# arcosoph/nanowakeword

Hardware: AMD Instinct MI355X
Metric: clips/sec (1 s @16 kHz PCM->logits) (higher is better)
Workload: dtype f32; 1 GPU; cnn head on (101,64) log-mel, batch=4096/GPU, 1 s 16 kHz mono int16 clips, 64-mel 25 ms/10 ms center frontend, fused STFT+mel HIP kernel, fp32; clips_per_gpu=4096, n_samples=16000, parallelism=batch-split x1

## Files before the change

### nanowakeword_amd/csrc/fe_steps.h

```cpp
#pragma once
#include <math.h>
#include <stdint.h>

#if defined(__HIPCC__)
#include <hip/hip_runtime.h>
#define NWW_HD __host__ __device__ __forceinline__
typedef float2 nww_c32;
#else
#define NWW_HD inline
struct nww_c32 { float x, y; };
#endif

#define FE_NFFT 400
#define FE_M 200
#define FE_BINS 201
#define FE_PSTRIDE 209
#define FE_MAX_MELS 128
#define FE_MAX_MELW 640

NWW_HD nww_c32 c_make(float x, float y) { nww_c32 r; r.x = x; r.y = y; return r; }
NWW_HD nww_c32 c_add(nww_c32 a, nww_c32 b) { return c_make(a.x + b.x, a.y + b.y); }
NWW_HD nww_c32 c_sub(nww_c32 a, nww_c32 b) { return c_make(a.x - b.x, a.y - b.y); }
NWW_HD nww_c32 c_mul(nww_c32 a, nww_c32 b) { return c_make(a.x * b.x - a.y * b.y, a.x * b.y + a.y * b.x); }
NWW_HD nww_c32 c_mul_negi(nww_c32 a) { return c_make(a.y, -a.x); }
// ... 126 lines not shown
NWW_HD float fe_s4(int f, int j, const FeTables* tb, const float* pw) {
    const float* p = pw + f * FE_PSTRIDE + tb->mel_lo[j];
    const float* w = tb->melw + tb->mel_off[j];
    const int n = tb->mel_cnt[j];
    float acc = 0.0f;
    for (int i = 0; i < n; ++i) acc = fmaf(p[i], w[i], acc);
    return acc;
}

NWW_HD float fe_db(float mel, float amin, float mult) {
    return mult * log10f(fmaxf(mel, amin));
}

NWW_HD int fe_reflect(int s, int N) {
    if (s < 0) s = -s;
    if (s >= N) s = 2 * (N - 1) - s;
    return s;
}

#define FE2_G 8
#define FE2_FRAME_DW 400
#define FE2_PSHIFT(f) (4 * ((f) >> 1))
#define FE2_STAGE_OFF 216
#define FE2_MAX_TILES 8
#define FE2_MAX_STEPS 512

#define FE2_CHUNK 8
#define FE2_MAX_CHUNKS 64
struct Fe2MelPlan {
    int32_t ntiles;
    int32_t total_steps;
    int32_t nchunks;
    int32_t tile_k0[FE2_MAX_TILES];
    int32_t tile_nsteps[FE2_MAX_TILES];
    int32_t tile_first[FE2_MAX_TILES];
    uint32_t chunk_meta[FE2_MAX_CHUNKS];
    float b[FE2_MAX_STEPS * 64];
};

NWW_HD void fe2_s1(const uint32_t s[8], const nww_c32 win[8], const nww_c32 tw[7], nww_c32 z[8]) {
#pragma unroll
    for (int n1 = 0; n1 < 8; ++n1)
        z[n1] = c_make((float)(int16_t)(s[n1] & 0xffffu) * win[n1].x, (float)(int16_t)(s[n1] >> 16) * win[n1].y);
    dft8(z);
#pragma unroll
    for (int k1 = 1; k1 < 8; ++k1) z[k1] = c_mul(z[k1], tw[k1 - 1]);
}

NWW_HD float fe2_mel_planned(const Fe2MelPlan* pl, const float* p, int j) {
    const int t = j >> 4, n = j & 15;
    const int k0 = pl->tile_k0[t], ns = pl->tile_nsteps[t];
    const float* b = pl->b + (size_t)pl->tile_first[t] * 64 + n;
    float acc[2] = {0.0f, 0.0f};
    for (int s = 0; s < ns; ++s)
        for (int kk = 0; kk < 4; ++kk) acc[s & 1] = fmaf(p[k0 + 4 * s + kk], b[s * 64 + kk * 16], acc[s & 1]);
    return acc[0] + acc[1];
}
```

### nanowakeword_amd/csrc/fe_tables.cpp

```cpp
#include "fe_tables.h"
#include <cmath>
#include <cstring>

static const double kPi = 3.14159265358979323846;

void fe_default_window(int win_length, std::vector<float>& window) {
    window.resize(win_length);
    for (int n = 0; n < win_length; ++n)
        window[n] = (float)(0.5 - 0.5 * std::cos(2.0 * kPi * n / win_length));
}

void fe_default_melfb(const FeParams& p, std::vector<float>& fb) {
    const int n_freqs = p.n_fft / 2 + 1;
    fb.assign((size_t)n_freqs * p.n_mels, 0.f);
    const double m_min = 2595.0 * std::log10(1.0 + (double)p.f_min / 700.0);
    const double m_max = 2595.0 * std::log10(1.0 + (double)p.f_max / 700.0);
    std::vector<double> f_pts(p.n_mels + 2);
    for (int i = 0; i < p.n_mels + 2; ++i) {
        const double m = m_min + (m_max - m_min) * i / (p.n_mels + 1);
        f_pts[i] = 700.0 * (std::pow(10.0, m / 2595.0) - 1.0);
    }
    const double nyq = (double)(p.sample_rate / 2);
    for (int k = 0; k < n_freqs; ++k) {
        const double f = nyq * k / (n_freqs - 1);
// ... 66 lines not shown
            for (int n = 0; n < 16; ++n) {
                const int j = 16 * t + n;
                if (j < p.n_mels && fb[(size_t)k * p.n_mels + j] != 0.f) { if (k < lo) lo = k; if (k > hi) hi = k; }
            }
        if (hi < 0) { lo = 0; hi = 0; }
        int ns = (hi - lo + 1 + 3) / 4;
        ns = (ns + FE2_CHUNK - 1) / FE2_CHUNK * FE2_CHUNK;
        if (first + ns > FE2_MAX_STEPS || (first + ns) / FE2_CHUNK > FE2_MAX_CHUNKS) return "mel filterbank is too dense for the MFMA plan";
        for (int c = 0; c < ns / FE2_CHUNK; ++c)
            pl->chunk_meta[first / FE2_CHUNK + c] =
                (uint32_t)(lo + 4 * FE2_CHUNK * c) | ((uint32_t)t << 12) | ((c == ns / FE2_CHUNK - 1) ? 1u << 16 : 0u);
        pl->tile_k0[t] = lo; pl->tile_nsteps[t] = ns; pl->tile_first[t] = first;
        for (int s = 0; s < ns; ++s)
            for (int l = 0; l < 64; ++l) {
                const int k = lo + 4 * s + (l >> 4), j = 16 * t + (l & 15);
                pl->b[(size_t)(first + s) * 64 + l] = (k < FE_BINS && j < p.n_mels) ? fb[(size_t)k * p.n_mels + j] : 0.f;
            }
        first += ns;
    }
    pl->total_steps = first;
    pl->nchunks = first / FE2_CHUNK;
    return "";
}
```

### nanowakeword_amd/csrc/fe_tables.h

```cpp
#pragma once
#include <string>
#include <vector>
#include "fe_steps.h"

struct FeParams {
    int sample_rate = 16000, n_fft = 400, win_length = 400, hop = 160, n_mels = 64, center = 1;
    float f_min = 0.f, f_max = 8000.f, amin = 1e-10f, db_mult = 10.f;
};

void fe_default_window(int win_length, std::vector<float>& window);
void fe_default_melfb(const FeParams& p, std::vector<float>& fb);

std::string fe_build_tables(const FeParams& p, const float* window, const float* fb, FeTables* out);

std::string fe2_build_mel_plan(const FeParams& p, const float* fb, Fe2MelPlan* out);

int fe_num_frames(const FeParams& p, int n_samples);
```

### nanowakeword_amd/csrc/frontend.h

```cpp
#pragma once
#include <hip/hip_runtime.h>
#include "fe_tables.h"

int fe2_lds_bytes(int waves, int mel_mode);
struct Fe2Sub {
    int nr = 0;
    int t0[4] = {0, 0, 0, 0}, t1[4] = {0, 0, 0, 0};
    int gend[4] = {0, 0, 0, 0};
    int ring_rows = 0, row0 = 0;
    size_t out_clip_stride = 0;
};
bool fe2_subset_supported(const FeParams& p, int mel_mode);
hipError_t fe2_launch(const int16_t* d_pcm, size_t row_stride, int B, int N, int T, const FeParams& p,
                      const FeTables* d_tables, const Fe2MelPlan* d_plan, float* d_db, float* d_mel, int frames_major,
                      int mel_mode, int max_taps, int block, int max_grid, hipStream_t stream, const Fe2Sub* subset = nullptr);
```

### nanowakeword_amd/csrc/frontend2.hip

```cpp
#include <hip/hip_runtime.h>
#include <stdlib.h>
#include "fe_steps.h"
#include "frontend.h"
#include "layers.h"

typedef float f32x4 __attribute__((ext_vector_type(4)));

struct Fe2MelLds {
    uint32_t desc[FE_MAX_MELS];
    float w[FE_MAX_MELW];
};

__device__ __forceinline__ void fe2_wave_sync() {
    __builtin_amdgcn_fence(__ATOMIC_RELEASE, "wavefront");
    __builtin_amdgcn_wave_barrier();
    __builtin_amdgcn_fence(__ATOMIC_ACQUIRE, "wavefront");
}

__device__ __forceinline__ void fe2_load_column(const int16_t* __restrict__ x, int base, int n2, uint32_t v[8]) {
    const uint32_t* p = reinterpret_cast<const uint32_t*>(x + base) + n2;
#pragma unroll
    for (int n1 = 0; n1 < 8; ++n1) v[n1] = p[25 * n1];
}

__device__ __forceinline__ float fe2_db(float mel, float amin, float mult, float floor_db) {
    const float db = (mult * 0.30102999566398120f) * __log2f(fmaxf(mel, amin));
    return mel > amin ? db : floor_db;
}

#define FE2_PARAMS                                                                                                      \
    const int16_t *__restrict__ pcm, size_t row_stride, int B, int N, int T, int ngroups, int hop, int pad, int n_mels,    \
        float amin, float db_mult, float floor_db, const FeTables *__restrict__ gtb, const Fe2MelPlan *__restrict__ plan,  \
        float *__restrict__ out_db, float *__restrict__ out_mel, int frames_major, int dbg, int gsz, Fe2Sub sub
#define FE2_ARGS pcm, row_stride, B, N, T, ngroups, hop, pad, n_mels, amin, db_mult, floor_db, gtb, plan, out_db, out_mel, frames_major, dbg, gsz, sub
template <int MEL, int FAST_OUT, int MAXT, bool RING>
__device__ __forceinline__ void fe2_wave_body(FE2_PARAMS) {
    extern __shared__ __attribute__((aligned(16))) char smem[];
    constexpr int MFMA_MEL = MEL == 1;
    const int lane = threadIdx.x & 63;
    const int wv = __builtin_amdgcn_readfirstlane((int)(threadIdx.x >> 6));
    const int nwv = blockDim.x >> 6;
    const int tb_bytes = MEL == 0 ? (int)sizeof(Fe2MelLds) : 0;
    Fe2MelLds* mt = reinterpret_cast<Fe2MelLds*>(smem);
    float* slab = reinterpret_cast<float*>(smem + tb_bytes) + wv * (FE2_G * FE2_FRAME_DW);
    if (MEL == 0) {
        for (int i = threadIdx.x; i < FE_MAX_MELS; i += blockDim.x)
            mt->desc[i] = (uint32_t)gtb->mel_lo[i] | ((uint32_t)gtb->mel_cnt[i] << 8) | ((uint32_t)gtb->mel_off[i] << 16);
        for (int i = threadIdx.x; i < FE_MAX_MELW; i += blockDim.x) mt->w[i] = gtb->melw[i];
        __syncthreads();
    }
    const int n2 = lane % 25, slot = lane / 25;
    nww_c32 win[8], tw[7];
#pragma unroll
    for (int n1 = 0; n1 < 8; ++n1) win[n1] = gtb->win2[25 * n1 + n2];
#pragma unroll
    for (int k1 = 1; k1 < 8; ++k1) tw[k1 - 1] = gtb->tw200[k1 * 25 + n2];
    const int k3a = lane, k3b = 64 + lane;
    const bool has_b = k3b <= 100;
    const nww_c32 twa = gtb->tw400[k3a], twb = gtb->tw400[has_b ? k3b : 100];
    const int ia2 = k3a ? FE_M - k3a : 0;
    const int f2 = lane >> 3, k1_2 = lane & 7;
    int co_off[4];
#pragma unroll
    for (int r = 0; r < 4; ++r) {
        const int i = 4 * lane + 256 * r, f = i / n_mels, j = i - f * n_mels;
        co_off[r] = f * FE2_FRAME_DW + FE2_STAGE_OFF + FE2_PSHIFT(f) + j;
    }
    const int mel_l5 = lane & 31;
    const int mel_j = (lane & 32) + ((mel_l5 < 4) ? mel_l5 : (mel_l5 < 12) ? 12 + mel_l5 : (mel_l5 < 16) ? mel_l5 - 8 : (mel_l5 < 20) ? 8 + mel_l5
                                     : (mel_l5 < 28) ? mel_l5 - 12 : mel_l5);
    float wreg[MAXT];
    int mel_lo_lane = 0;
    if (MEL == 2) {
        const int j = min(mel_j, n_mels - 1);
        const int lo = gtb->mel_lo[j], sh4 = lo & 3;
        mel_lo_lane = lo - sh4;
        const int cnt = mel_j < n_mels ? gtb->mel_cnt[j] : 0, off = gtb->mel_off[j];
#pragma unroll
        for (int i = 0; i < MAXT; ++i) wreg[i] = (i >= sh4 && i - sh4 < cnt) ? gtb->melw[off + i - sh4] : 0.0f;
    }
    const int mel_nchunks = MFMA_MEL ? plan->nchunks : 0;
    const uint32_t mel_meta = MFMA_MEL ? plan->chunk_meta[lane] : 0u;
    const bool aligned = ((reinterpret_cast<uintptr_t>(pcm) | (row_stride * sizeof(int16_t))) & 3) == 0;

    const int total = B * ngroups;
    const int stride = gridDim.x * nwv;
    uint32_t cur[8];
    auto geom = [&](int item, int& b, int& t0, int& nf) {
        b = item / ngroups;
        const int g = item - b * ngroups;
        if (!RING || sub.nr == 0) {
            t0 = g * gsz;
            nf = min(gsz, T - t0);
        } else {
            int r = 0;
            while (r + 1 < sub.nr && g >= sub.gend[r]) ++r;
            t0 = sub.t0[r] + (g - (r ? sub.gend[r - 1] : 0)) * gsz;
            nf = min(gsz, sub.t1[r] - t0);
        }
    };
    auto interior = [&](int t0, int nf) {
        const int s0 = t0 * hop - pad;
// ... 40 lines not shown
#pragma unroll
                    for (int n1 = 0; n1 < 8; ++n1) nxt[n1] = span[((fn * hop) >> 1) + n2 + 25 * n1];
                }
            }
            if (slot < 2 && f < nf && !(dbg & 1)) {
                nww_c32 z[8];
                fe2_s1(cur, win, tw, z);
                nww_c32* y = reinterpret_cast<nww_c32*>(slab + f * FE2_FRAME_DW) + n2;
#pragma unroll
                for (int k1 = 0; k1 < 8; ++k1) y[k1 * 25] = z[k1];
            }
#pragma unroll
            for (int n1 = 0; n1 < 8; ++n1) cur[n1] = nxt[n1];
        }
        fe2_wave_sync();
        if (f2 < nf && !(dbg & 2)) {
            nww_c32* zf = reinterpret_cast<nww_c32*>(slab + f2 * FE2_FRAME_DW);
            const nww_c32* row = zf + k1_2 * 25;
            nww_c32* dst = zf + k1_2;
            dft25<true>([&](int i) { return row[i]; }, [&](int i, nww_c32 v) { dst[8 * i] = v; });
        }
        fe2_wave_sync();
        if (item + stride < total) prefetch_first(item + stride);
        if (!(dbg & 4)) {
            const nww_c32* z0 = reinterpret_cast<const nww_c32*>(slab);
            nww_c32 a1 = z0[k3a], b1 = z0[ia2], a2 = z0[has_b ? k3b : 0], b2 = z0[has_b ? FE_M - k3b : 0];
#pragma unroll
            for (int f = 0; f < FE2_G; ++f) {
                if (f >= nf) break;
                nww_c32 na1 = a1, nb1 = b1, na2 = a2, nb2 = b2;
                if (f + 1 < FE2_G) {
                    const nww_c32* zn = reinterpret_cast<const nww_c32*>(slab + (f + 1) * FE2_FRAME_DW);
                    na1 = zn[k3a]; nb1 = zn[ia2]; na2 = zn[has_b ? k3b : 0]; nb2 = zn[has_b ? FE_M - k3b : 0];
                }
                float pa1, pb1, pa2, pb2;
                fe_s3_core(a1, b1, twa, &pa1, &pb1);
                fe_s3_core(a2, b2, twb, &pa2, &pb2);
                float* p = slab + f * FE2_FRAME_DW + FE2_PSHIFT(f);
                p[k3a] = pa1;
                p[FE_M - k3a] = pb1;
                if (has_b) { p[k3b] = pa2; p[FE_M - k3b] = pb2; }
                a1 = na1; b1 = nb1; a2 = na2; b2 = nb2;
            }
        }
        fe2_wave_sync();
        if (!(dbg & 8)) {
// ... 37 lines not shown
                                            const size_t o = ((size_t)b * n_mels + j) * T + t0 + f;
                                            if (out_db) out_db[o] = db;
                                            if (out_mel) out_mel[o] = m;
                                        }
                                    }
                                }
                            }
                        }
                        acc0 = f32x4{0.f, 0.f, 0.f, 0.f};
                        acc1 = f32x4{0.f, 0.f, 0.f, 0.f};
                    }
                };
                float a0[FE2_CHUNK], b0[FE2_CHUNK], a1[FE2_CHUNK], b1[FE2_CHUNK];
                const int last = mel_nchunks - 1;
                load_chunk(0, a0, b0);
#pragma unroll 1
                for (int c = 0; c < mel_nchunks; c += 2) {
                    load_chunk(min(c + 1, last), a1, b1);
                    run_chunk(c, a0, b0);
                    load_chunk(min(c + 2, last), a0, b0);
                    if (c + 1 < mel_nchunks) run_chunk(c + 1, a1, b1);
                }
            } else if (MEL == 2) {
                const float* p0 = slab + mel_lo_lane;
#pragma unroll 1
                for (int f = 0; f < nf; f += 2) {
                    const float* pa = p0 + f * FE2_FRAME_DW + FE2_PSHIFT(f);
                    const float* pb = pa + FE2_FRAME_DW;
                    float ma = 0.0f, mb = 0.0f;
#pragma unroll
                    for (int i = 0; i < MAXT; i += 4) {
                        const float4 a4 = *reinterpret_cast<const float4*>(__builtin_assume_aligned(pa + i, 16));
                        const float4 b4 = *reinterpret_cast<const float4*>(__builtin_assume_aligned(pb + i, 16));
                        ma = fmaf(a4.x, wreg[i], ma); mb = fmaf(b4.x, wreg[i], mb);
                        ma = fmaf(a4.y, wreg[i + 1], ma); mb = fmaf(b4.y, wreg[i + 1], mb);
                        ma = fmaf(a4.z, wreg[i + 2], ma); mb = fmaf(b4.z, wreg[i + 2], mb);
                        ma = fmaf(a4.w, wreg[i + 3], ma); mb = fmaf(b4.w, wreg[i + 3], mb);
                    }
                    if (mel_j < n_mels) {
                        const float da = fe2_db(ma, amin, db_mult, floor_db), db2 = fe2_db(mb, amin, db_mult, floor_db);
                        if (FAST_OUT) {
                            float* st = slab + f * FE2_FRAME_DW + FE2_STAGE_OFF + FE2_PSHIFT(f) + mel_j;
                            st[0] = da;
                            st[FE2_FRAME_DW] = db2;
                        } else {
#pragma unroll
                            for (int q = 0; q < 2; ++q) {
                                const int fq = f + q;
                                const float m = q ? mb : ma, db = q ? db2 : da;
                                if (fq < nf) {
                                    if (frames_major) {
                                        slab[fq * FE2_FRAME_DW + FE2_STAGE_OFF + FE2_PSHIFT(fq) + mel_j] = db;
                                        if (out_mel) out_mel[((size_t)b * T + t0 + fq) * n_mels + mel_j] = m;
                                    } else {
                                        const size_t o = ((size_t)b * n_mels + mel_j) * T + t0 + fq;
                                        if (out_db) out_db[o] = db;
                                        if (out_mel) out_mel[o] = m;
                                    }
                                }
                            }
                        }
                    }
                }
            } else {
                const int f = lane & 7;
                if (f < nf) {
                    const float* prow = slab + f * FE2_FRAME_DW + FE2_PSHIFT(f);
                    for (int j = lane >> 3; j < n_mels; j += 8) {
                        const uint32_t d = mt->desc[j];
                        const float* p = prow + (d & 0xffu);
                        const float* w = mt->w + (d >> 16);
                        const int n = (d >> 8) & 0xffu;
                        float m = 0.0f;
                        for (int i = 0; i < n; ++i) m = fmaf(p[i], w[i], m);
                        const float db = fe2_db(m, amin, db_mult, floor_db);
                        if (frames_major) {
                            slab[f * FE2_FRAME_DW + FE2_STAGE_OFF + FE2_PSHIFT(f) + j] = db;
                            if (out_mel) out_mel[((size_t)b * T + t0 + f) * n_mels + j] = m;
                        } else {
                            const size_t o = ((size_t)b * n_mels + j) * T + t0 + f;
                            if (out_db) out_db[o] = db;
// ... 24 lines not shown
                }
            } else {
                for (int i = lane; i < cnt; i += 64) {
                    const int f = i / n_mels, j = i - f * n_mels;
                    dst[i] = slab[f * FE2_FRAME_DW + FE2_STAGE_OFF + FE2_PSHIFT(f) + j];
                }
            }
            }
        }
        fe2_wave_sync();
    }
}

template <int MEL, int FAST_OUT, int MAXT, bool RING = false>
__global__ void __launch_bounds__(256, 3) fe2_wave_kernel(FE2_PARAMS) { fe2_wave_body<MEL, FAST_OUT, MAXT, RING>(FE2_ARGS); }

bool fe2_subset_supported(const FeParams& p, int mel_mode) { return mel_mode != 0 && (p.n_mels & 3) == 0; }

int fe2_lds_bytes(int waves, int mel_mode) {
    return waves * FE2_G * FE2_FRAME_DW * 4 + (mel_mode == 0 ? (int)sizeof(Fe2MelLds) : 0);
}

hipError_t fe2_launch(const int16_t* d_pcm, size_t row_stride, int B, int N, int T, const FeParams& p,
                      const FeTables* d_tables, const Fe2MelPlan* d_plan, float* d_db, float* d_mel, int frames_major,
                      int mel_mode, int max_taps, int block, int max_grid, hipStream_t stream, const Fe2Sub* subset) {
    if (block < 64 || block > 1024 || (block & 63)) return hipErrorInvalidValue;
    const int nwv = block / 64;
    Fe2Sub sub = subset ? *subset : Fe2Sub{};
    if (sub.nr < 0 || sub.nr > 4) return hipErrorInvalidValue;
    if ((sub.nr || sub.ring_rows) && !(frames_major && d_db && !d_mel && (p.n_mels & 3) == 0)) return hipErrorInvalidValue;
    if (sub.ring_rows && (sub.ring_rows < T || sub.row0 < 0 || sub.row0 >= sub.ring_rows)) return hipErrorInvalidValue;
    auto count_groups = [&](int g) {
        if (sub.nr == 0) return (T + g - 1) / g;
        int n = 0;
        for (int r = 0; r < sub.nr; ++r) { n += (sub.t1[r] - sub.t0[r] + g - 1) / g; sub.gend[r] = n; }
        return n;
    };
    for (int r = 0; r < sub.nr; ++r)
        if (sub.t0[r] < 0 || sub.t1[r] <= sub.t0[r] || sub.t1[r] > T) return hipErrorInvalidValue;
    int ngroups = count_groups(FE2_G);
    int mode = mel_mode;
    if (mode == 2 && (p.n_mels > 64 || max_taps > 25)) mode = 1;
    const int lds = fe2_lds_bytes(nwv, mode);
    const int fast = (frames_major && d_db && !d_mel) ? 1 : 0;
    const bool ring = sub.nr > 0 || sub.ring_rows > 0;
    if (ring && (mode == 0 || !fast)) return hipErrorInvalidValue;
    auto kern = mode == 0 ? fe2_wave_kernel<0, 0, 1>
              : mode == 1 ? (ring ? fe2_wave_kernel<1, 1, 1, true> : fast ? fe2_wave_kernel<1, 1, 1> : fe2_wave_kernel<1, 0, 1>)
              : max_taps <= 17 ? (ring ? fe2_wave_kernel<2, 1, 20, true> : fast ? fe2_wave_kernel<2, 1, 20> : fe2_wave_kernel<2, 0, 20>)
                               : (ring ? fe2_wave_kernel<2, 1, 28, true> : fast ? fe2_wave_kernel<2, 1, 28> : fe2_wave_kernel<2, 0, 28>);
    const void* fn = reinterpret_cast<const void*>(kern);
    {
        hipError_t e = nww_allow_lds(fn, (size_t)lds);
        if (e != hipSuccess) return e;
    }
#ifdef NWW_ABLATION
    static const int dbg = [] { const char* e = getenv("NWW_FE_DBG"); return e ? atoi(e) : 0; }();
#else
    const int dbg = 0;
#endif
    const int small_g = 2;
    int gsz = FE2_G;
    if (mode == 2 && small_g >= 2 && small_g < FE2_G && (small_g % 2) == 0 && (long long)B * ngroups * 4 <= (long long)max_grid * nwv) {
        gsz = small_g;
        ngroups = count_groups(gsz);
    }
    const long long total = (long long)B * ngroups;
    long long need = (total + nwv - 1) / nwv;
    int grid = (int)(need < max_grid ? need : max_grid);
    if (grid < 1) grid = 1;
    const int pad = p.center ? FE_NFFT / 2 : 0;
    hipLaunchKernelGGL(kern, dim3(grid), dim3(block), lds, stream, d_pcm, row_stride, B, N, T, ngroups, p.hop, pad, p.n_mels,
                       p.amin, p.db_mult, p.db_mult * log10f(p.amin), d_tables, d_plan, d_db, d_mel, frames_major, dbg, gsz, sub);
    return hipGetLastError();
}
```

### nanowakeword_amd/csrc/nww_api.hip

```cpp
#include "nww_internal.h"

static hipEvent_t prof_event(nww_handle* h) {
    hipEvent_t e = nullptr;
    if (!h->event_pool.empty()) { e = h->event_pool.back(); h->event_pool.pop_back(); return e; }
    if (hipEventCreate(&e) != hipSuccess) return nullptr;
    return e;
}
void nww_prof_mark(nww_handle* h, hipStream_t s, int id_of_next) {
    if (!h->profiling || !h->prof_active) return;
    hipEvent_t e = prof_event(h);
    if (!e) return;
    (void)hipEventRecord(e, s);
    h->prof_runs.back().push_back(e);
    h->prof_ids.back().push_back(id_of_next);
}
void nww_prof_begin(nww_handle* h) {
    if (!h->profiling) return;
    h->prof_active = (h->prof_counter++ % h->prof_period) == 0;
    if (!h->prof_active) return;
    h->prof_runs.emplace_back();
    h->prof_ids.emplace_back();
}

static thread_local std::string g_create_err;
// ... 98 lines not shown
        if (p) (void)hipFree(p);
    h->d_ws = nullptr; h->d_pcm = nullptr; h->d_logmel = nullptr; h->d_feats = nullptr; h->d_emb = nullptr;
    h->d_hid = nullptr; h->d_logits = nullptr; h->d_probs = nullptr; h->d_splitk = nullptr; h->cap_B = 0; h->cap_N = 0;
}

extern "C" int nww_stream_close(nww_handle* h);

extern "C" int nww_emb_close(nww_handle* h);
extern "C" int nww_comm_destroy(nww_handle* h);
extern "C" int nww_destroy(nww_handle* h) {
    if (!h) return NWW_OK;
    (void)hipSetDevice(h->cfg.device);
    free_ws(h);
    nww_stream_close(h);
    nww_emb_close(h);
    nww_comm_destroy(h);
    if (h->pin_in) (void)hipHostFree(h->pin_in);
    if (h->pin_out) (void)hipHostFree(h->pin_out);
    if (h->d_weights) (void)hipFree(h->d_weights);
    for (auto& kv : h->x3_weights) (void)hipFree(kv.second);
    for (void* d : h->packed_weights) (void)hipFree(d);
    if (h->d_tables) (void)hipFree(h->d_tables);
    if (h->d_melplan) (void)hipFree(h->d_melplan);
    if (h->own_stream) (void)hipStreamDestroy(h->own_stream);
    for (auto& run : h->prof_runs) for (auto e : run) (void)hipEventDestroy(e);
    for (auto e : h->event_pool) (void)hipEventDestroy(e);
    delete h;
    return NWW_OK;
}

extern "C" int nww_num_tensors(const nww_handle* h) { return h ? (int)h->keys.size() : 0; }

extern "C" int nww_tensor_info(const nww_handle* h, int32_t i, const char** key, int64_t* shape4, int32_t* ndim) {
    if (!h || i < 0 || i >= (int)h->keys.size()) return NWW_ERR_INVALID;
    const std::string& k = h->keys[i];
    const HostTensor& t = h->tensors.at(k);
    if (key) *key = k.c_str();
    if (ndim) *ndim = (int)t.shape.size();
    if (shape4) for (size_t d = 0; d < 4; ++d) shape4[d] = d < t.shape.size() ? t.shape[d] : 1;
    return NWW_OK;
}

extern "C" int nww_load_tensor(nww_handle* h, const char* key, const void* host, const int64_t* shape, int32_t ndim,
                               int32_t dtype) {
    if (!h || !key || !host || !shape || ndim < 0) return fail(h, NWW_ERR_INVALID, "nww_load_tensor: null argument");
    if (h->finalized) return fail(h, NWW_ERR_STATE, "nww_load_tensor('%s') after nww_finalize", key);
// ... 147 lines not shown
    if (d_probs && r.need_sigmoid) {
        nww_prof_mark(h, s, id);
        hipError_t e = launch_unary(r.logits, d_probs, (size_t)B, ACT_SIGMOID, s);
        if (e != hipSuccess) return fail(h, NWW_ERR_HIP, "launch 'sigmoid' failed: %s", hipGetErrorString(e));
    }
    nww_prof_mark(h, s, -1);
    if (done_armed) *done_armed = r.done_armed;
    return NWW_OK;
}

int nww_check_run(nww_handle* h, int B) {
    if (!h) return NWW_ERR_INVALID;
    if (!h->finalized) return fail(h, NWW_ERR_STATE, "model not finalized: call nww_finalize after loading the state_dict");
    if (B <= 0) return fail(h, NWW_ERR_INVALID, "batch must be positive (got %d)", B);
    return NWW_OK;
}

int nww_frontend_on_dev(nww_handle* h, const int16_t* d_pcm, int B, int N, float* d_db, float* d_mel, int frames_major,
                        hipStream_t s, int* frames_out, size_t row_stride, const Fe2Sub* sub) {
    const int T = fe_num_frames(h->fe, N);
    if (T <= 0) return fail(h, NWW_ERR_INVALID, "clip of %d samples is too short for n_fft=%d (center=%d)", N, h->fe.n_fft, h->fe.center);
    if (frames_out) *frames_out = T;
    static const int mel_env = 2;
    hipError_t e = fe2_launch(d_pcm, row_stride ? row_stride : (size_t)N, B, N, T, h->fe, h->d_tables, h->d_melplan, d_db, d_mel, frames_major, mel_env, h->mel_max_taps, 256, h->cu_count * 3, s, sub);
    if (e != hipSuccess) return fail(h, NWW_ERR_HIP, "frontend launch failed: %s", hipGetErrorString(e));
    return NWW_OK;
}

extern "C" int nww_frontend_dev(nww_handle* h, const int16_t* d_pcm, int32_t B, int32_t N, float* d_logmel,
                                int32_t frames_major, void* stream) {
    int rc = nww_check_run(h, B);
    if (rc) return rc;
    if (!d_pcm || !d_logmel) return fail(h, NWW_ERR_INVALID, "null device pointer");
    HIP_TRY(h, hipSetDevice(h->cfg.device));
    return nww_frontend_on_dev(h, d_pcm, B, N, d_logmel, nullptr, frames_major, stream ? (hipStream_t)stream : h->own_stream, nullptr);
}

int nww_forward_pcm_on_dev(nww_handle* h, const int16_t* d_pcm, int B, int N, float* d_logits, float* d_probs, hipStream_t s,
                           size_t row_stride, unsigned int* done_flag, unsigned int done_seq, bool* done_armed) {
    const nww_config& c = h->cfg;
    const int T = fe_num_frames(h->fe, N);
    if (T <= 0) return fail(h, NWW_ERR_INVALID, "clip of %d samples is too short for n_fft=%d (center=%d)", N, h->fe.n_fft, h->fe.center);
    const int rows = c.mel_major_features ? c.n_mels : T, cols = c.mel_major_features ? T : c.n_mels;
    if (rows != c.in_rows || cols != c.in_cols)
        return fail(h, NWW_ERR_SHAPE, "frontend yields (%d,%d) features for %d samples but the head was built for input_shape=(%d,%d)",
                    rows, cols, N, c.in_rows, c.in_cols);
    int rc = nww_ensure_ws(h, B, N);
// ... 205 lines not shown
```

### nanowakeword_amd/csrc/nww_internal.h

```cpp
#pragma once
#include <hip/hip_runtime.h>
#include <atomic>
#include <cmath>
#include <cstdarg>
#include <cstdio>
#include <cstdlib>
#include <cstring>
#include <functional>
#include <map>
#include <string>
#include <vector>

#include "../../include/nww.h"
#include "fe_tables.h"
#include "frontend.h"
#include "layers.h"
#include "trunk.h"
#include "ffn_x3.h"
#include "lin_x3.h"
#include "attn_x3.h"
#include "dual_x3.h"
#include "emb_stream.h"
#include "tcn_x3.h"

// ... 29 lines not shown
    bool need_sigmoid = true;
    unsigned int* done_flag = nullptr; unsigned int done_seq = 0; bool done_armed = false;
    float* splitk_ws = nullptr; size_t splitk_floats = 0; int cu_count = 256;
    struct { bool active = false; int out_id = 0, parts = 0; size_t stride = 0; const float *bias = nullptr, *alpha = nullptr, *beta = nullptr; int act = 0; } deferred;
};


struct X3Key {
    const float* w; int fmt; float scale;
    bool operator<(const X3Key& o) const { return w != o.w ? w < o.w : fmt != o.fmt ? fmt < o.fmt : scale < o.scale; }
};

struct nww_handle {
    bool e2e_transposed = false;
    nww_config cfg;
    FeParams fe;
    std::string err;
    std::vector<std::string> keys;
    std::map<std::string, HostTensor> tensors;
    bool finalized = false;
    float* d_weights = nullptr;
    FeTables* d_tables = nullptr;
    Fe2MelPlan* d_melplan = nullptr;
    int mel_max_taps = 0;
    hipStream_t own_stream = nullptr;
    std::vector<Step> plan;
    size_t buf_per_clip[6] = {0, 0, 0, 0, 0, 0};
    int cap_B = 0, cap_N = 0;
    bool trunk_blocked = false;
    int cap_rows = 0;
    float* d_ws = nullptr;
    int16_t* d_pcm = nullptr;
    float* d_logmel = nullptr;
    float* d_feats = nullptr;
    float* d_emb = nullptr;
    float* d_hid = nullptr;
    float* d_logits = nullptr;
    float* d_probs = nullptr;
    float* d_splitk = nullptr;
    int16_t* d_ring = nullptr; int16_t* d_chunk = nullptr;
    std::string plan_error;
    bool clamps_features = false;
    bool x_stride_ok = false;
    bool stream_conv = false;
    int stream_H = 0, stream_W = 0;
    bool inc_fe = false, inc_conv = false, primed = false;
    float* d_lm_ring = nullptr; int lm_rows = 0, lm_pos = 0, lm_shift = 0, fe_edge_l = 0, fe_edge_r = 0;
// ... 66 lines not shown
```

### nanowakeword_amd/csrc/nww_plan.hip

```cpp
#include "nww_internal.h"
#include "bc_chain.h"

const Knobs& nww_knobs() {
    static const Knobs k = [] {
        auto env = [](const char* name, int d) { const char* e = getenv(name); return e ? atoi(e) : d; };
        Knobs r;
        r.trunk = env("NWW_TRUNK", 1); r.conv_mfma = env("NWW_CONV_MFMA", 1); r.conv3_x3 = env("NWW_CONV3_X3", 1);
        r.gemm_x3 = env("NWW_GEMM_X3", 1); r.lin_x3 = env("NWW_LIN_X3", 1); r.ffn_fused = env("NWW_FFN_FUSED", 1);
        r.attn_fused = env("NWW_ATTN_FUSED", 1); r.mha_mfma = env("NWW_MHA_MFMA", 1); r.bc_front = env("NWW_BC_FRONT", 1);
        r.bc_chain = env("NWW_BC_CHAIN", 1); r.tail = env("NWW_TAIL", 1); r.stream_inc = env("NWW_STREAM_INC", 3);
        r.f16_range_log2 = env("NWW_F16_RANGE_LOG2", 16);
        return r;
    }();
    return k;
}

namespace {
using Shape = std::vector<int64_t>;
struct SpecBuilder {
    std::vector<std::string>& keys;
    std::map<std::string, HostTensor>& t;
    void add(const std::string& k, Shape s) { keys.push_back(k); t[k].shape = std::move(s); }
    void lin(const std::string& p, int out, int in) { add(p + ".weight", {out, in}); add(p + ".bias", {out}); }
    void ln(const std::string& p, int d) { add(p + ".weight", {d}); add(p + ".bias", {d}); }
// ... 643 lines not shown
    }
    HIP_TRY(h, hipMalloc(&h->d_weights, (total + 4) * sizeof(float)));
    for (auto& kv : h->tensors) {
        if (!kv.second.loaded || kv.first.rfind("frontend.", 0) == 0) continue;
        HIP_TRY(h, hipMemcpy(h->d_weights + kv.second.dev_off, kv.second.data.data(), kv.second.data.size() * sizeof(float),
                             hipMemcpyHostToDevice));
    }
    return NWW_OK;
}

int build_frontend_tables(nww_handle* h) {
    std::vector<float> win, fb;
    auto wi = h->tensors.find("frontend.window");
    if (wi != h->tensors.end() && wi->second.loaded) win = wi->second.data; else fe_default_window(h->fe.win_length, win);
    auto fi = h->tensors.find("frontend.mel_fb");
    if (fi != h->tensors.end() && fi->second.loaded) fb = fi->second.data; else fe_default_melfb(h->fe, fb);
    FeTables tb;
    const std::string e = fe_build_tables(h->fe, win.data(), fb.data(), &tb);
    if (!e.empty()) return fail(h, NWW_ERR_INVALID, "frontend tables: %s", e.c_str());
    const size_t tbytes = (sizeof(FeTables) + 15) & ~(size_t)15;
    HIP_TRY(h, hipMalloc(&h->d_tables, tbytes));
    HIP_TRY(h, hipMemset(h->d_tables, 0, tbytes));
    HIP_TRY(h, hipMemcpy(h->d_tables, &tb, sizeof(FeTables), hipMemcpyHostToDevice));
    h->mel_max_taps = 0;
    for (int j = 0; j < h->fe.n_mels; ++j) h->mel_max_taps = tb.mel_cnt[j] > h->mel_max_taps ? tb.mel_cnt[j] : h->mel_max_taps;
    std::vector<Fe2MelPlan> plan(1);
    const std::string e2 = fe2_build_mel_plan(h->fe, fb.data(), plan.data());
    if (!e2.empty()) return fail(h, NWW_ERR_INVALID, "frontend mel plan: %s", e2.c_str());
    HIP_TRY(h, hipMalloc(&h->d_melplan, sizeof(Fe2MelPlan)));
    HIP_TRY(h, hipMemcpy(h->d_melplan, plan.data(), sizeof(Fe2MelPlan), hipMemcpyHostToDevice));
    return NWW_OK;
}

bool add_attn_x3(PlanCtx& p, const std::string& q, int hb, int T, int D, int NH) {
    if (!(nww_knobs().attn_fused && p.h->f16 && p.h->conv_products == 6 && attn_x3_supported(T, D, NH))) return false;
    const float *iw = p.W(q + ".attention.in_proj_weight"), *ib = p.W(q + ".attention.in_proj_bias");
    const float *ow = p.W(q + ".attention.out_proj.weight"), *ob = p.W(q + ".attention.out_proj.bias");
    const auto hiw = f16_fetch(p.h, iw, (size_t)3 * D * D), how = f16_fetch(p.h, ow, (size_t)D * D);
    const float ws_in = f16_wscale(hiw), ws_out = f16_wscale(how);
    auto l1max = [&](int r0) {
        double worst = 0;
        for (int r = r0; r < r0 + D; ++r) {
            double t = 0;
            for (int k = 0; k < D; ++k) t += std::fabs((double)hiw[(size_t)r * D + k]);
            worst = std::fmax(worst, t);
        }
        return worst;
    };
// ... 771 lines not shown
```

Before: 9.300 million clips/s.

## Pack two mel filters per lane with host-built pair plan for register mel stage

```diff
diff --git a/nanowakeword_amd/csrc/fe_steps.h b/nanowakeword_amd/csrc/fe_steps.h
--- a/nanowakeword_amd/csrc/fe_steps.h
+++ b/nanowakeword_amd/csrc/fe_steps.h
@@ -172,6 +172,7 @@
 #define FE2_FRAME_DW 400
 #define FE2_PSHIFT(f) (4 * ((f) >> 1))
 #define FE2_STAGE_OFF 216
+#define FE2_STAGE_SPARE 100
 #define FE2_MAX_TILES 8
 #define FE2_MAX_STEPS 512
 
@@ -188,6 +189,19 @@
     float b[FE2_MAX_STEPS * 64];
 };
 
+#define FE2_PAIR_WAVES 12
+#define FE2_PAIR_MAXW 32
+struct Fe2PairPlan {
+    int32_t sx, sy;
+    int32_t maxt;
+    int32_t lane_a[64], lane_b[64];
+    int32_t lane_par[64];
+    int32_t lane_flex[64];
+    int32_t bin_f[64], bin_x[64], bin_y[64];
+    float w[64][FE2_PAIR_MAXW];
+    int32_t rt[FE2_PAIR_WAVES][64][8];
+};
+
 NWW_HD void fe2_s1(const uint32_t s[8], const nww_c32 win[8], const nww_c32 tw[7], nww_c32 z[8]) {
 #pragma unroll
     for (int n1 = 0; n1 < 8; ++n1)
diff --git a/nanowakeword_amd/csrc/fe_tables.cpp b/nanowakeword_amd/csrc/fe_tables.cpp
--- a/nanowakeword_amd/csrc/fe_tables.cpp
+++ b/nanowakeword_amd/csrc/fe_tables.cpp
@@ -112,3 +112,115 @@
     pl->nchunks = first / FE2_CHUNK;
     return "";
 }
+
+int fe2_filter_chunks(const FeTables* tb, int j) {
+    const int cnt = tb->mel_cnt[j];
+    return cnt > 0 ? ((tb->mel_lo[j] & 3) + cnt + 3) / 4 : 0;
+}
+
+namespace {
+struct Pair { int a, b; };
+
+bool pair_filters(const FeTables* tb, int n_mels, int sx, int sy, std::vector<Pair>& pairs) {
+    std::vector<int> order(n_mels), ch(n_mels);
+    for (int j = 0; j < n_mels; ++j) { order[j] = j; ch[j] = fe2_filter_chunks(tb, j); }
+    for (int i = 1; i < n_mels; ++i)
+        for (int k = i; k > 0 && ch[order[k]] > ch[order[k - 1]]; --k) { const int t = order[k]; order[k] = order[k - 1]; order[k - 1] = t; }
+    std::vector<char> used(n_mels, 0);
+    pairs.clear();
+    for (int i = 0; i < n_mels; ++i) {
+        const int a = order[i];
+        if (used[a]) continue;
+        used[a] = 1;
+        if (ch[a] > sx + 1) return false;
+        const int room = ch[a] == sx + 1 ? sy : sy + 1;
+        int b = -1;
+        for (int k = i + 1; k < n_mels && b < 0; ++k)
+            if (!used[order[k]] && ch[order[k]] <= room) b = order[k];
+        if (b >= 0) used[b] = 1;
+        pairs.push_back({a, b});
+    }
+    return pairs.size() <= 32;
+}
+
+int lane_position(int lane) {
+    const int l5 = lane & 31;
+    return (lane & 32) + (l5 < 4 ? l5 : l5 < 12 ? 12 + l5 : l5 < 16 ? l5 - 8 : l5 < 20 ? 8 + l5 : l5 < 28 ? l5 - 12 : l5);
+}
+}
+
+std::string fe2_build_pair_plan(const FeParams& p, const FeTables* tb, Fe2PairPlan* pl) {
+    std::memset(pl, 0, sizeof(*pl));
+    if (p.n_mels <= 0 || p.n_mels > 64) return "the register-filter mel stage takes n_mels <= 64";
+    const int n = p.n_mels;
+    static const int shapes[2][2] = {{4, 1}, {6, 1}};
+    std::vector<Pair> pairs;
+    int sx = 0, sy = 0, maxt = 0;
+    for (int s = 0; s < 2 && !maxt; ++s)
+        if (pair_filters(tb, n, shapes[s][0], shapes[s][1], pairs)) { sx = shapes[s][0]; sy = shapes[s][1]; maxt = 4 * (1 + sx + sy); }
+    if (!maxt) {
+        int widest = 0;
+        for (int j = 0; j < n; ++j) widest = fe2_filter_chunks(tb, j) > widest ? fe2_filter_chunks(tb, j) : widest;
+        bool ok = false;
+        for (int steps = 1; steps <= 2 * widest + 1 && !ok; ++steps)
+            for (sy = 0; sy < steps && !ok; ++sy) { sx = steps - 1 - sy; ok = sx >= sy && pair_filters(tb, n, sx, sy, pairs); if (ok) break; }
+        if (!ok) return "no lane assignment for the mel filterbank";
+    }
+    pl->sx = sx; pl->sy = sy; pl->maxt = maxt;
+    for (size_t i = 1; i < pairs.size(); ++i)
+        for (size_t k = i; k > 0 && tb->mel_lo[pairs[k].a] < tb->mel_lo[pairs[k - 1].a]; --k) { const Pair t = pairs[k]; pairs[k] = pairs[k - 1]; pairs[k - 1] = t; }
+    auto weight = [&](int j, int bin) {
+        const int i = bin - tb->mel_lo[j];
+        return (j >= 0 && i >= 0 && i < tb->mel_cnt[j]) ? tb->melw[tb->mel_off[j] + i] : 0.0f;
+    };
+    for (int lane = 0; lane < 64; ++lane) {
+        const int pos = lane_position(lane), g = pos >> 4, pi = (g >> 1) * 16 + (pos & 15);
+        pl->lane_a[lane] = pl->lane_b[lane] = -1;
+        pl->lane_par[lane] = g & 1;
+        const int fa = (g & 1) * FE2_FRAME_DW, fb = FE2_FRAME_DW - fa;
+        auto addresses = [&]() {
+            const int a = pl->lane_a[lane], b = pl->lane_b[lane], flex = pl->lane_flex[lane];
+            for (int v = 0; v < FE2_PAIR_WAVES; ++v) {
+                const int slab = v * FE2_G * FE2_FRAME_DW;
+                int32_t* r = pl->rt[v][lane];
+                r[0] = 4 * (slab + pl->bin_f[lane] + (flex ? fa : fb));
+                r[1] = 4 * (slab + pl->bin_x[lane] + fa);
+                r[2] = 4 * (slab + pl->bin_y[lane] + fb);
+                r[3] = (g & 1) | (flex ? (int32_t)0x80000000u : 0);
+                r[4] = 4 * (slab + fa + FE2_STAGE_OFF + (a >= 0 ? a : FE2_STAGE_SPARE));
+                r[5] = 4 * (slab + fb + FE2_STAGE_OFF + (b >= 0 ? b : FE2_STAGE_SPARE));
+                r[6] = a; r[7] = b;
+            }
+        };
+        if (pi >= (int)pairs.size()) { addresses(); continue; }
+        const int a = pairs[pi].a, b = pairs[pi].b;
+        const int flex = fe2_filter_chunks(tb, a) == sx + 1;
+        const int a0 = tb->mel_lo[a] & ~3, b0 = b >= 0 ? tb->mel_lo[b] & ~3 : 0;
+        pl->lane_a[lane] = a; pl->lane_b[lane] = b; pl->lane_flex[lane] = flex;
+        pl->bin_f[lane] = flex ? a0 : b0;
+        pl->bin_x[lane] = flex ? a0 + 4 : a0;
+        pl->bin_y[lane] = flex ? b0 : b0 + 4;
+        addresses();
+        if (!maxt) continue;
+        float* w = pl->w[lane];
+        for (int i = 0; i < 4; ++i) w[i] = flex ? weight(a, a0 + i) : (b >= 0 ? weight(b, b0 + i) : 0.0f);
+        for (int i = 0; i < 4 * sx; ++i) w[4 + i] = weight(a, pl->bin_x[lane] + i);
+        for (int i = 0; i < 4 * sy; ++i) w[4 + 4 * sx + i] = b >= 0 ? weight(b, pl->bin_y[lane] + i) : 0.0f;
+    }
+    return "";
+}
+
+extern "C" int fe2_pair_plan_query(int n_mels, const float* fb, int32_t* out) {
+    FeParams p; p.n_mels = n_mels;
+    std::vector<float> w, f;
+    fe_default_window(p.win_length, w);
+    if (!fb) { fe_default_melfb(p, f); fb = f.data(); }
+    FeTables tb;
+    std::vector<Fe2PairPlan> pl(1);
+    if (!fe_build_tables(p, w.data(), fb, &tb).empty() || !fe2_build_pair_plan(p, &tb, pl.data()).empty()) return -1;
+    out[0] = pl[0].sx; out[1] = pl[0].sy; out[2] = pl[0].maxt;
+    for (int l = 0; l < 64; ++l) {
+        out[3 + l] = pl[0].lane_a[l]; out[67 + l] = pl[0].lane_b[l]; out[131 + l] = pl[0].lane_par[l]; out[195 + l] = pl[0].lane_flex[l];
+    }
+    return 0;
+}
diff --git a/nanowakeword_amd/csrc/fe_tables.h b/nanowakeword_amd/csrc/fe_tables.h
--- a/nanowakeword_amd/csrc/fe_tables.h
+++ b/nanowakeword_amd/csrc/fe_tables.h
@@ -15,4 +15,7 @@
 
 std::string fe2_build_mel_plan(const FeParams& p, const float* fb, Fe2MelPlan* out);
 
+std::string fe2_build_pair_plan(const FeParams& p, const FeTables* tb, Fe2PairPlan* out);
+int fe2_filter_chunks(const FeTables* tb, int j);
+
 int fe_num_frames(const FeParams& p, int n_samples);
diff --git a/nanowakeword_amd/csrc/frontend.h b/nanowakeword_amd/csrc/frontend.h
--- a/nanowakeword_amd/csrc/frontend.h
+++ b/nanowakeword_amd/csrc/frontend.h
@@ -12,5 +12,5 @@
 };
 bool fe2_subset_supported(const FeParams& p, int mel_mode);
 hipError_t fe2_launch(const int16_t* d_pcm, size_t row_stride, int B, int N, int T, const FeParams& p,
-                      const FeTables* d_tables, const Fe2MelPlan* d_plan, float* d_db, float* d_mel, int frames_major,
-                      int mel_mode, int max_taps, int block, int max_grid, hipStream_t stream, const Fe2Sub* subset = nullptr);
+                      const FeTables* d_tables, const Fe2MelPlan* d_plan, const Fe2PairPlan* d_pair, int pair_maxt, float* d_db, float* d_mel,
+                      int frames_major, int mel_mode, int block, int max_grid, hipStream_t stream, const Fe2Sub* subset = nullptr);
diff --git a/nanowakeword_amd/csrc/frontend2.hip b/nanowakeword_amd/csrc/frontend2.hip
--- a/nanowakeword_amd/csrc/frontend2.hip
+++ b/nanowakeword_amd/csrc/frontend2.hip
@@ -31,8 +31,8 @@
 #define FE2_PARAMS                                                                                                      \
     const int16_t *__restrict__ pcm, size_t row_stride, int B, int N, int T, int ngroups, int hop, int pad, int n_mels,    \
         float amin, float db_mult, float floor_db, const FeTables *__restrict__ gtb, const Fe2MelPlan *__restrict__ plan,  \
-        float *__restrict__ out_db, float *__restrict__ out_mel, int frames_major, int dbg, int gsz, Fe2Sub sub
-#define FE2_ARGS pcm, row_stride, B, N, T, ngroups, hop, pad, n_mels, amin, db_mult, floor_db, gtb, plan, out_db, out_mel, frames_major, dbg, gsz, sub
+        const Fe2PairPlan *__restrict__ pair, float *__restrict__ out_db, float *__restrict__ out_mel, int frames_major, int dbg, int gsz, Fe2Sub sub
+#define FE2_ARGS pcm, row_stride, B, N, T, ngroups, hop, pad, n_mels, amin, db_mult, floor_db, gtb, plan, pair, out_db, out_mel, frames_major, dbg, gsz, sub
 template <int MEL, int FAST_OUT, int MAXT, bool RING>
 __device__ __forceinline__ void fe2_wave_body(FE2_PARAMS) {
     extern __shared__ __attribute__((aligned(16))) char smem[];
@@ -66,18 +66,13 @@
         const int i = 4 * lane + 256 * r, f = i / n_mels, j = i - f * n_mels;
         co_off[r] = f * FE2_FRAME_DW + FE2_STAGE_OFF + FE2_PSHIFT(f) + j;
     }
-    const int mel_l5 = lane & 31;
-    const int mel_j = (lane & 32) + ((mel_l5 < 4) ? mel_l5 : (mel_l5 < 12) ? 12 + mel_l5 : (mel_l5 < 16) ? mel_l5 - 8 : (mel_l5 < 20) ? 8 + mel_l5
-                                     : (mel_l5 < 28) ? mel_l5 - 12 : mel_l5);
+    constexpr int SX = MAXT / 4 - 2;
+    constexpr int WRES = MAXT > 24 ? 24 : MAXT;
     float wreg[MAXT];
-    int mel_lo_lane = 0;
+    const int mel_rt_off = (wv * 64 + lane) * 32;
     if (MEL == 2) {
-        const int j = min(mel_j, n_mels - 1);
-        const int lo = gtb->mel_lo[j], sh4 = lo & 3;
-        mel_lo_lane = lo - sh4;
-        const int cnt = mel_j < n_mels ? gtb->mel_cnt[j] : 0, off = gtb->mel_off[j];
-#pragma unroll
-        for (int i = 0; i < MAXT; ++i) wreg[i] = (i >= sh4 && i - sh4 < cnt) ? gtb->melw[off + i - sh4] : 0.0f;
+#pragma unroll
+        for (int i = 0; i < WRES; ++i) wreg[i] = pair->w[lane][i];
     }
     const int mel_nchunks = MFMA_MEL ? plan->nchunks : 0;
     const uint32_t mel_meta = MFMA_MEL ? plan->chunk_meta[lane] : 0u;
@@ -164,6 +159,19 @@
         }
         fe2_wave_sync();
         if (item + stride < total) prefetch_first(item + stride);
+        int4 mel_r0 = {0, 0, 0, 0}, mel_r1 = {0, 0, 0, 0};
+        if (MEL == 2) {
+            int ro = mel_rt_off;
+            asm volatile("" : "+v"(ro));
+            const int4* rt = reinterpret_cast<const int4*>(reinterpret_cast<const char*>(pair->rt) + ro);
+            mel_r0 = rt[0];
+            mel_r1 = rt[1];
+#pragma unroll
+            for (int i = WRES; i < MAXT; i += 4) {
+                const float4 w4 = *reinterpret_cast<const float4*>(pair->w[lane] + i);
+                wreg[i] = w4.x; wreg[i + 1] = w4.y; wreg[i + 2] = w4.z; wreg[i + 3] = w4.w;
+            }
+        }
         if (!(dbg & 4)) {
             const nww_c32* z0 = reinterpret_cast<const nww_c32*>(slab);
             nww_c32 a1 = z0[k3a], b1 = z0[ia2], a2 = z0[has_b ? k3b : 0], b2 = z0[has_b ? FE_M - k3b : 0];
@@ -247,41 +255,50 @@
                     if (c + 1 < mel_nchunks) run_chunk(c + 1, a1, b1);
                 }
             } else if (MEL == 2) {
-                const float* p0 = slab + mel_lo_lane;
-#pragma unroll 1
-                for (int f = 0; f < nf; f += 2) {
-                    const float* pa = p0 + f * FE2_FRAME_DW + FE2_PSHIFT(f);
-                    const float* pb = pa + FE2_FRAME_DW;
-                    float ma = 0.0f, mb = 0.0f;
-#pragma unroll
-                    for (int i = 0; i < MAXT; i += 4) {
-                        const float4 a4 = *reinterpret_cast<const float4*>(__builtin_assume_aligned(pa + i, 16));
-                        const float4 b4 = *reinterpret_cast<const float4*>(__builtin_assume_aligned(pb + i, 16));
-                        ma = fmaf(a4.x, wreg[i], ma); mb = fmaf(b4.x, wreg[i], mb);
-                        ma = fmaf(a4.y, wreg[i + 1], ma); mb = fmaf(b4.y, wreg[i + 1], mb);
-                        ma = fmaf(a4.z, wreg[i + 2], ma); mb = fmaf(b4.z, wreg[i + 2], mb);
-                        ma = fmaf(a4.w, wreg[i + 3], ma); mb = fmaf(b4.w, wreg[i + 3], mb);
-                    }
-                    if (mel_j < n_mels) {
-                        const float da = fe2_db(ma, amin, db_mult, floor_db), db2 = fe2_db(mb, amin, db_mult, floor_db);
-                        if (FAST_OUT) {
-                            float* st = slab + f * FE2_FRAME_DW + FE2_STAGE_OFF + FE2_PSHIFT(f) + mel_j;
-                            st[0] = da;
-                            st[FE2_FRAME_DW] = db2;
-                        } else {
-#pragma unroll
-                            for (int q = 0; q < 2; ++q) {
-                                const int fq = f + q;
-                                const float m = q ? mb : ma, db = q ? db2 : da;
-                                if (fq < nf) {
-                                    if (frames_major) {
-                                        slab[fq * FE2_FRAME_DW + FE2_STAGE_OFF + FE2_PSHIFT(fq) + mel_j] = db;
-                                        if (out_mel) out_mel[((size_t)b * T + t0 + fq) * n_mels + mel_j] = m;
-                                    } else {
-                                        const size_t o = ((size_t)b * n_mels + mel_j) * T + t0 + fq;
-                                        if (out_db) out_db[o] = db;
-                                        if (out_mel) out_mel[o] = m;
-                                    }
+                const float *mel_pf = reinterpret_cast<const float*>(smem + mel_r0.x), *mel_px = reinterpret_cast<const float*>(smem + mel_r0.y),
+                            *mel_py = reinterpret_cast<const float*>(smem + mel_r0.z);
+                float *mel_sa = reinterpret_cast<float*>(smem + mel_r1.x), *mel_sb = reinterpret_cast<float*>(smem + mel_r1.y);
+                const bool mel_flex = mel_r0.w < 0;
+#pragma unroll(FAST_OUT ? FE2_G / 2 : 1)
+                for (int f = 0; f < FE2_G; f += 2) {
+                    if (f >= nf) break;
+                    const int o = f * FE2_FRAME_DW + FE2_PSHIFT(f);
+                    float mz = 0.0f;
+                    {
+                        const float4 p4 = *reinterpret_cast<const float4*>(__builtin_assume_aligned(mel_pf + o, 16));
+                        mz = fmaf(p4.x, wreg[0], mz); mz = fmaf(p4.y, wreg[1], mz); mz = fmaf(p4.z, wreg[2], mz); mz = fmaf(p4.w, wreg[3], mz);
+                    }
+                    float ma = mel_flex ? mz : 0.0f, mb = mel_flex ? 0.0f : mz;
+#pragma unroll
+                    for (int i = 0; i < SX; ++i) {
+                        const float4 p4 = *reinterpret_cast<const float4*>(__builtin_assume_aligned(mel_px + o + 4 * i, 16));
+                        const float* w = wreg + 4 + 4 * i;
+                        ma = fmaf(p4.x, w[0], ma); ma = fmaf(p4.y, w[1], ma); ma = fmaf(p4.z, w[2], ma); ma = fmaf(p4.w, w[3], ma);
+                    }
+                    {
+                        const float4 p4 = *reinterpret_cast<const float4*>(__builtin_assume_aligned(mel_py + o, 16));
+                        const float* w = wreg + 4 + 4 * SX;
+                        mb = fmaf(p4.x, w[0], mb); mb = fmaf(p4.y, w[1], mb); mb = fmaf(p4.z, w[2], mb); mb = fmaf(p4.w, w[3], mb);
+                    }
+                    const float da = fe2_db(ma, amin, db_mult, floor_db), db2 = fe2_db(mb, amin, db_mult, floor_db);
+                    if (FAST_OUT) {
+                        mel_sa[o] = da;
+                        mel_sb[o] = db2;
+                    } else {
+#pragma unroll
+                        for (int q = 0; q < 2; ++q) {
+                            const int j = q ? mel_r1.w : mel_r1.z;
+                            const int fq = f + ((mel_r0.w ^ q) & 1);
+                            float* st = q ? mel_sb : mel_sa;
+                            const float m = q ? mb : ma, db = q ? db2 : da;
+                            if (j >= 0 && fq < nf) {
+                                if (frames_major) {
+                                    st[o] = db;
+                                    if (out_mel) out_mel[((size_t)b * T + t0 + fq) * n_mels + j] = m;
+                                } else {
+                                    const size_t oo = ((size_t)b * n_mels + j) * T + t0 + fq;
+                                    if (out_db) out_db[oo] = db;
+                                    if (out_mel) out_mel[oo] = m;
                                 }
                             }
                         }
@@ -352,8 +369,8 @@
 }
 
 hipError_t fe2_launch(const int16_t* d_pcm, size_t row_stride, int B, int N, int T, const FeParams& p,
-                      const FeTables* d_tables, const Fe2MelPlan* d_plan, float* d_db, float* d_mel, int frames_major,
-                      int mel_mode, int max_taps, int block, int max_grid, hipStream_t stream, const Fe2Sub* subset) {
+                      const FeTables* d_tables, const Fe2MelPlan* d_plan, const Fe2PairPlan* d_pair, int pair_maxt, float* d_db, float* d_mel,
+                      int frames_major, int mel_mode, int block, int max_grid, hipStream_t stream, const Fe2Sub* subset) {
     if (block < 64 || block > 1024 || (block & 63)) return hipErrorInvalidValue;
     const int nwv = block / 64;
     Fe2Sub sub = subset ? *subset : Fe2Sub{};
@@ -370,15 +387,15 @@
         if (sub.t0[r] < 0 || sub.t1[r] <= sub.t0[r] || sub.t1[r] > T) return hipErrorInvalidValue;
     int ngroups = count_groups(FE2_G);
     int mode = mel_mode;
-    if (mode == 2 && (p.n_mels > 64 || max_taps > 25)) mode = 1;
+    if (mode == 2 && (p.n_mels > 64 || !d_pair || (pair_maxt != 24 && pair_maxt != 32) || nwv > FE2_PAIR_WAVES)) mode = 1;
     const int lds = fe2_lds_bytes(nwv, mode);
     const int fast = (frames_major && d_db && !d_mel) ? 1 : 0;
     const bool ring = sub.nr > 0 || sub.ring_rows > 0;
     if (ring && (mode == 0 || !fast)) return hipErrorInvalidValue;
-    auto kern = mode == 0 ? fe2_wave_kernel<0, 0, 1>
-              : mode == 1 ? (ring ? fe2_wave_kernel<1, 1, 1, true> : fast ? fe2_wave_kernel<1, 1, 1> : fe2_wave_kernel<1, 0, 1>)
-              : max_taps <= 17 ? (ring ? fe2_wave_kernel<2, 1, 20, true> : fast ? fe2_wave_kernel<2, 1, 20> : fe2_wave_kernel<2, 0, 20>)
-                               : (ring ? fe2_wave_kernel<2, 1, 28, true> : fast ? fe2_wave_kernel<2, 1, 28> : fe2_wave_kernel<2, 0, 28>);
+    auto kern = mode == 0 ? fe2_wave_kernel<0, 0, 24>
+              : mode == 1 ? (ring ? fe2_wave_kernel<1, 1, 24, true> : fast ? fe2_wave_kernel<1, 1, 24> : fe2_wave_kernel<1, 0, 24>)
+              : pair_maxt == 24 ? (ring ? fe2_wave_kernel<2, 1, 24, true> : fast ? fe2_wave_kernel<2, 1, 24> : fe2_wave_kernel<2, 0, 24>)
+                                : (ring ? fe2_wave_kernel<2, 1, 32, true> : fast ? fe2_wave_kernel<2, 1, 32> : fe2_wave_kernel<2, 0, 32>);
     const void* fn = reinterpret_cast<const void*>(kern);
     {
         hipError_t e = nww_allow_lds(fn, (size_t)lds);
@@ -401,6 +418,6 @@
     if (grid < 1) grid = 1;
     const int pad = p.center ? FE_NFFT / 2 : 0;
     hipLaunchKernelGGL(kern, dim3(grid), dim3(block), lds, stream, d_pcm, row_stride, B, N, T, ngroups, p.hop, pad, p.n_mels,
-                       p.amin, p.db_mult, p.db_mult * log10f(p.amin), d_tables, d_plan, d_db, d_mel, frames_major, dbg, gsz, sub);
+                       p.amin, p.db_mult, p.db_mult * log10f(p.amin), d_tables, d_plan, d_pair, d_db, d_mel, frames_major, dbg, gsz, sub);
     return hipGetLastError();
 }
diff --git a/nanowakeword_amd/csrc/nww_api.hip b/nanowakeword_amd/csrc/nww_api.hip
--- a/nanowakeword_amd/csrc/nww_api.hip
+++ b/nanowakeword_amd/csrc/nww_api.hip
@@ -144,6 +144,7 @@
     for (void* d : h->packed_weights) (void)hipFree(d);
     if (h->d_tables) (void)hipFree(h->d_tables);
     if (h->d_melplan) (void)hipFree(h->d_melplan);
+    if (h->d_pairplan) (void)hipFree(h->d_pairplan);
     if (h->own_stream) (void)hipStreamDestroy(h->own_stream);
     for (auto& run : h->prof_runs) for (auto e : run) (void)hipEventDestroy(e);
     for (auto e : h->event_pool) (void)hipEventDestroy(e);
@@ -337,7 +338,7 @@
     if (T <= 0) return fail(h, NWW_ERR_INVALID, "clip of %d samples is too short for n_fft=%d (center=%d)", N, h->fe.n_fft, h->fe.center);
     if (frames_out) *frames_out = T;
     static const int mel_env = 2;
-    hipError_t e = fe2_launch(d_pcm, row_stride ? row_stride : (size_t)N, B, N, T, h->fe, h->d_tables, h->d_melplan, d_db, d_mel, frames_major, mel_env, h->mel_max_taps, 256, h->cu_count * 3, s, sub);
+    hipError_t e = fe2_launch(d_pcm, row_stride ? row_stride : (size_t)N, B, N, T, h->fe, h->d_tables, h->d_melplan, h->d_pairplan, h->mel_pair_maxt, d_db, d_mel, frames_major, mel_env, 256, h->cu_count * 3, s, sub);
     if (e != hipSuccess) return fail(h, NWW_ERR_HIP, "frontend launch failed: %s", hipGetErrorString(e));
     return NWW_OK;
 }
diff --git a/nanowakeword_amd/csrc/nww_internal.h b/nanowakeword_amd/csrc/nww_internal.h
--- a/nanowakeword_amd/csrc/nww_internal.h
+++ b/nanowakeword_amd/csrc/nww_internal.h
@@ -75,7 +75,8 @@
     float* d_weights = nullptr;
     FeTables* d_tables = nullptr;
     Fe2MelPlan* d_melplan = nullptr;
-    int mel_max_taps = 0;
+    Fe2PairPlan* d_pairplan = nullptr;
+    int mel_pair_maxt = 0;
     hipStream_t own_stream = nullptr;
     std::vector<Step> plan;
     size_t buf_per_clip[6] = {0, 0, 0, 0, 0, 0};
diff --git a/nanowakeword_amd/csrc/nww_plan.hip b/nanowakeword_amd/csrc/nww_plan.hip
--- a/nanowakeword_amd/csrc/nww_plan.hip
+++ b/nanowakeword_amd/csrc/nww_plan.hip
@@ -689,8 +689,15 @@
     HIP_TRY(h, hipMalloc(&h->d_tables, tbytes));
     HIP_TRY(h, hipMemset(h->d_tables, 0, tbytes));
     HIP_TRY(h, hipMemcpy(h->d_tables, &tb, sizeof(FeTables), hipMemcpyHostToDevice));
-    h->mel_max_taps = 0;
-    for (int j = 0; j < h->fe.n_mels; ++j) h->mel_max_taps = tb.mel_cnt[j] > h->mel_max_taps ? tb.mel_cnt[j] : h->mel_max_taps;
+    h->mel_pair_maxt = 0;
+    if (h->fe.n_mels <= 64) {
+        std::vector<Fe2PairPlan> pair(1);
+        const std::string e3 = fe2_build_pair_plan(h->fe, &tb, pair.data());
+        if (!e3.empty()) return fail(h, NWW_ERR_INVALID, "frontend pair plan: %s", e3.c_str());
+        HIP_TRY(h, hipMalloc(&h->d_pairplan, sizeof(Fe2PairPlan)));
+        HIP_TRY(h, hipMemcpy(h->d_pairplan, pair.data(), sizeof(Fe2PairPlan), hipMemcpyHostToDevice));
+        h->mel_pair_maxt = pair[0].maxt;
+    }
     std::vector<Fe2MelPlan> plan(1);
     const std::string e2 = fe2_build_mel_plan(h->fe, fb.data(), plan.data());
     if (!e2.empty()) return fail(h, NWW_ERR_INVALID, "frontend mel plan: %s", e2.c_str());
```

Result: no change. 9.362 million clips/s, median of 6 (+0.7%).
